# dimalit/ipt

Measured on AMD Instinct MI355X. Metric: Mpaths/sec at 1024^2, 8-bounce, sample_scenes[0]; achieved HBM GB/s, higher is better.
Workload: dtype f32; 1 GPU; c2: box 1024x1024, 1280 spp, depth_max 8, n_rays 16; width=1024, height=1024, spp=1280, depth_max=8, n_rays=16, tile_rows=0, calls=queued (ipt_render_device_async), one wait, parallelism=tiles1, per_rank=the whole frame's tiles dealt round-robin; 256 x N passes per step (weak)

## Files before the change

### ipt_amd/csrc/ipt_kernels.hip

```cpp
#include <hip/hip_runtime.h>

#include <algorithm>
#include <array>
#include <cmath>
#include <cstdio>
#include <cstdlib>
#include <cstring>
#include <strings.h>
#include <mutex>
#include <string>
#include <thread>
#include <type_traits>
#include <vector>

#include "../../include/ipt_capi.h"
#include "ipt_bvh.h"
#include "ipt_internal.h"
#include "ipt_path.h"
#include "ipt_knobs.h"
#include "ipt_diag.h"

using namespace ipt;

namespace {
// ... 52 lines not shown
    const int* __restrict__ grid_idx;
    const BvhNode* __restrict__ bvh_nodes;
    const BvhSphere* __restrict__ bvh_prims;
    int n_nodes;
    const BvhNode* __restrict__ light_nodes;
    int n_light_nodes;
    int lnodes_lds;
    const int* __restrict__ lgrid;
    const float4* __restrict__ lax;
    int lg_nu, lg_nv;
    float lg_u0, lg_v0, lg_icw, lg_ich;
    float lg_e;
    unsigned long long pk_u0, pk_u1, sa_u;
    int sa_on;
    float sa_pz, sa_nz;
    float sa_cl;
    float lg_pn, lg_nn;
    int cdf_bsearch;
    int cdf_p2;
    float cdf_p2s, cdf_end;
    int cdf_p2e;
    uint32_t cdf_end_t;
    int lpf_calc, lc_shift;
    float lc_x0, lc_y0, lc_dx, lc_dy, lc_ax, lc_ay;
    int ltr_calc, lg_ident;
    float lc_ix, lc_iy, lc_area, lc_spow;
    const int* __restrict__ cdf_lo;
    double inv_per_pass, inv_w;
    uint32_t per_pass32;
    int box_inrange;
    const float* __restrict__ cos_a;
    const float2* __restrict__ cos_b;
    const float2* __restrict__ frame_sc;
    const uint4* __restrict__ rg;
    int count;
};

__host__ __device__ inline uint32_t udiv_exact(uint32_t n, uint32_t d, double inv_d) {
    uint32_t q = (uint32_t)((double)n * inv_d);
    if (n - q * d >= d) ++q;
    return q;
}
__device__ __forceinline__ bool longer_sq(float x, float y) {
    const bool far_gt = x > y * 1.000001907f && y >= 1e-30f;
    const bool le = x <= y;
    const bool tie = !far_gt && !le;
    bool r = far_gt;
    if (__builtin_expect(__any(tie), 0))
        if (tie) r = sqrt_(x) > sqrt_(y);
    return r;
}
__device__ __forceinline__ bool longer(vec3 a, vec3 b) { return longer_sq(dot(a, a), dot(b, b)); }

__device__ __forceinline__ void vgpr_hold(float& f) { asm volatile("" : "+v"(f)); }
__device__ __forceinline__ void vgpr_hold(vec3& v) { vgpr_hold(v.x); vgpr_hold(v.y); vgpr_hold(v.z); }
__device__ __forceinline__ void vgpr_hold(int& i) { asm volatile("" : "+v"(i)); }

constexpr uint32_t kFrameTabLo = 0x3b800000u;
constexpr uint32_t kFrameTabSpan = 0x04000000u;
constexpr size_t kFrameTabEntries = 2 * ((size_t)kFrameTabSpan + 1);
__device__ __forceinline__ void frame_sc_lookup(const float2* __restrict__ tab, vec3 to, float& s, float& c) {
    const uint32_t u = f2u(to.z), m = u & 0x7fffffffu;
    const bool in = m - kFrameTabLo <= kFrameTabSpan;
    if (in) {
        const float2 e = tab[((m - kFrameTabLo) << 1) | (u >> 31)];
        s = e.x;
        c = e.y;
    }
    if (__builtin_expect(__any(!in), 0))
        if (!in) frame_angle_sc(to, &s, &c);
}

__device__ __forceinline__ bool owned_row(const KParams& kp, int yi) {
    if (kp.n_shards <= 1 || kp.tile_rows <= 0) return true;
    return ((yi / kp.tile_rows) % kp.n_shards) == kp.shard_id;
}

struct Win8 {
    uint32_t a0, a1, a2, a3, b0, b1, b2, b3;
};

__device__ __forceinline__ uint32_t sel4(uint32_t j, uint32_t x0, uint32_t x1, uint32_t x2, uint32_t x3) {
    const bool b0 = (j & 1u) != 0u, b1 = (j & 2u) != 0u;
    const uint32_t lo = b0 ? x1 : x0, hi = b0 ? x3 : x2;
    return b1 ? hi : lo;
}

__device__ __forceinline__ uint32_t cdf_threshold24(float c) {
    const float x = c * 16777216.0f;
    return !(x > 0.0f) ? 0u : (x >= 16777216.0f ? 16777216u : (uint32_t)__builtin_ceilf(x));
}

__device__ __forceinline__ void philox_fill(uint32_t& d0, uint32_t& d1, uint32_t& d2, uint32_t& d3,
                                            uint32_t blk, uint32_t pass, uint32_t pix, uint32_t k0,
                                            uint32_t k1) {
    u32x4 o = philox4x32_10(blk, pass, pix, 0u, k0, k1);
    d0 = o.v[0];
    d1 = o.v[1];
    d2 = o.v[2];
    d3 = o.v[3];
}

__device__ __forceinline__ float bvh_box_entry(const BvhNode& b, vec3 o, vec3 inv) {
    const float tx0 = (b.bmin[0] - o.x) * inv.x, tx1 = (b.bmax[0] - o.x) * inv.x;
    const float ty0 = (b.bmin[1] - o.y) * inv.y, ty1 = (b.bmax[1] - o.y) * inv.y;
    const float tz0 = (b.bmin[2] - o.z) * inv.z, tz1 = (b.bmax[2] - o.z) * inv.z;
// ... 856 lines not shown
    LightSet<LMODE> LS;
    LS.lds = lights_lds;
    LS.glob = kp.lights;
    LS.wl = global_lights(LMODE) ? gl_lds : weights_lds;
    LS.cl = global_lights(LMODE) ? cdf_gl : cdf_lds;
    LS.wg = kp.weights;
    LS.cg = kp.cdf;
    if (one_light(LMODE)) {
        LS.one = kp.lights[0];
        if (IPT_LIGHT_HOLD && (IPT_RES_HOLD || !resumable_geom(GEOM))) {
            vgpr_hold(LS.one.P); vgpr_hold(LS.one.x); vgpr_hold(LS.one.y);
            vgpr_hold(LS.one.n); vgpr_hold(LS.one.inv.c[0]); vgpr_hold(LS.one.inv.c[1]); vgpr_hold(LS.one.inv.c[2]);
        }
        LS.w0 = kp.weights[0];
        LS.c0 = kp.cdf[0];
        LS.c1 = kp.cdf[1];
    }

    auto ltrace = [&](const LightDev& L, vec3 o, vec3 d, vec3* hp, vec3* hn) -> bool {
        if constexpr (LMODE == kLightsOneA10) return light_trace_ax<1, 0, IPT_LIGHT_INR>(L, o, d, hp, hn);
        else if constexpr (LMODE == kLightsOneA01) return light_trace_ax<0, 1, IPT_LIGHT_INR>(L, o, d, hp, hn);
        else if constexpr (grid_lights(LMODE) && lattice_a10(LMODE)) return light_trace_ax<1, 0, IPT_LIGHT_INR>(L, o, d, hp, hn);
        else if constexpr (grid_lights(LMODE)) return light_trace_ax<0, 1, IPT_LIGHT_INR>(L, o, d, hp, hn);
        else return light_trace<LMODE == kLightsAny>(L, o, d, hp, hn);
    };
    auto lpdf = [&](const LightDev& L, vec3 o, bool h, vec3 hp, vec3 hn) -> float {
        if constexpr (LMODE == kLightsOneA10 || LMODE == kLightsOneA01) return light_pdf_ax<2, IPT_LIGHT_INR>(L, o, h, hp, hn);
        else if constexpr (grid_lights(LMODE)) return light_pdf_ax<2, IPT_LIGHT_INR>(L, o, h, hp, hn);
        else return light_pdf(L, o, h, hp, hn);
    };
    auto lsample = [&](const LightDev& L, vec3 o, float a, float b) -> vec3 {
        if constexpr (LMODE == kLightsOneA10) return light_sample_dir_ax<1, 0, IPT_LIGHT_INR>(L, o, a, b);
        else if constexpr (LMODE == kLightsOneA01) return light_sample_dir_ax<0, 1, IPT_LIGHT_INR>(L, o, a, b);
        else if constexpr (grid_lights(LMODE) && lattice_a10(LMODE)) return light_sample_dir_ax<1, 0, IPT_LIGHT_INR>(L, o, a, b);
        else if constexpr (grid_lights(LMODE)) return light_sample_dir_ax<0, 1, IPT_LIGHT_INR>(L, o, a, b);
        else return light_sample_dir<LMODE == kLightsAny>(L, o, a, b);
    };

    KParams kg = kp;
    if (IPT_RES_HOLD && resumable_geom(GEOM)) {
        for (int a = 0; a < 3; ++a) {
            vgpr_hold(kg.grid_g0[a]);
            vgpr_hold(kg.grid_h[a]);
            vgpr_hold(kg.grid_n[a]);
        }
        vgpr_hold(kg.grid_m);
        vgpr_hold(kg.bvh_tmargin);
    }
    const int lane = tid & 63;
    const uint64_t lanemask_lt = (lane == 0) ? 0ull : (~0ull >> (64 - lane));
    const int nl = one_light(LMODE) ? 1 : kp.n_lights;
    const float w_sdf = kp.weights[nl];
    const unsigned long long per_pass = (unsigned long long)kp.n_cand * (unsigned long long)kp.W;
    const bool n_pow2 = kp.n_rays > 0 && (kp.n_rays & (kp.n_rays - 1)) == 0;
    const int n_log2 = n_pow2 ? 31 - __clz(kp.n_rays) : 0;

    __builtin_amdgcn_s_waitcnt(0);

    unsigned long long pool_next = 0, pool_end = 0;

    bool active = true, has_path = false, fresh = false, need_frame = false, need_b = false;
    int pick = -1;
    float u1 = 0.0f, u2 = 0.0f, tr = 0.0f, cs_c = 0.0f, cs_s = 0.0f;
    float pfs = 0.0f, pfc = 0.0f;
    vec3 pto = v3(0, 0, 0);
    bool pfok = false;
    uint32_t unit = 0;
    uint32_t rpass = 0, rpix = 0, k = 0, blk = 0;
    Win8 w;
    vec3 tpos = v3(0, 0, 0);
    int fdepth = -1;
    uint32_t finm = 0;
    constexpr bool kRes = resumable_geom(GEOM);
    constexpr bool kResL = resumable_lights(LMODE, GEOM);
    constexpr int kFramePf = (kRes || kResL) ? 0 : IPT_FRAME_PF;
    constexpr bool kSkipAhead = IPT_SKIP_AHEAD && (one_light(LMODE) || grid_lights(LMODE)) && !kResL;
    constexpr bool kPreSkip = kSkipAhead && IPT_PRE_SKIP && kFramePf == 3;
    bool tracing = false;
    float xlmix = 0.0f;
    vec3 xro = v3(0, 0, 0), xrd = v3(0, 0, 0), xli_pos = v3(0, 0, 0);
    int xrdepth = 0, xi = 0, xbidx = -1;
    float xli_y = 0.0f;
    bool xis_iter = false, xhas_li = false;
    float xmult = 0.0f, xli_pow = 0.0f, xbest = 0.0f;
    vec3 xtm = v3(0, 0, 0);
    float tres = 0.0f;
    int ti = 0, tdepth = 0, tkind = 0;
    uint32_t c_paths = 0, c_traced = 0, c_surf = 0, c_light = 0, c_exp = 0, c_iter = 0,
             c_lsamp = 0, c_skip = 0, c_sframe = 0, c_ltr = 0, c_drift = 0, c_nodes = 0, c_tests = 0,
             c_lnode = 0, c_ltest = 0;
    IPT_DIAG_STATE

    for (;;) {
        IPT_STAMP_AT(0);
        const bool need = active && !has_path;
        const uint64_t needmask = __ballot(need);
        if (needmask) {
            const int cnt = __popcll(needmask);
            const int rank = __popcll(needmask & lanemask_lt);
            unsigned long long avail = pool_end - pool_next;
            unsigned long long my = 0;
            if ((unsigned long long)cnt > avail) {
                unsigned long long base = 0;
                if (lane == __ffsll((long long)needmask) - 1) {
                    base = atomicAdd(kp.unit_counter, (unsigned long long)kPoolChunk);
                    if (kp.drained && base + kPoolChunk >= kp.total_units)
                        __hip_atomic_store(kp.drained, kp.drain_seq, __ATOMIC_RELAXED, __HIP_MEMORY_SCOPE_SYSTEM);
                }
                base = __shfl(base, __ffsll((long long)needmask) - 1);
                if ((unsigned long long)rank < avail)
                    my = pool_next + rank;
                else
                    my = base + (rank - avail);
                pool_next = base + (cnt - avail);
                pool_end = base + kPoolChunk;
            } else {
                my = pool_next + rank;
                pool_next += cnt;
            }
            if (need) {
                if (my >= kp.total_units) {
                    active = false;
                } else {
                    unit = (uint32_t)my;
                    has_path = true;
                    fresh = true;
                }
            }
        }

        IPT_STAMP_AT(1);
        if (active) { IPT_PHASE(0); }
        auto pop_node = [&]() {
        if (active && has_path && !fresh && !((kRes || kResL) && tracing) && ti >= (kp.n_rays >> tdepth)) {
            IPT_PHASE(1);
            auto fin_v = [&](float r, int d) {
                float v = 0.0f;
                if (isfinite_(r))
                    v = n_pow2 ? r * __builtin_amdgcn_ldexpf(1.0f, -(n_log2 - d)) : r / (float)(kp.n_rays >> d);
                return v;
            };
            const uint32_t m = ~finm & ((1u << tdepth) - 1u);
            const int stop = m ? 31 - (int)__clz(m) : -1;
            auto lvl = [&](int l) { return stk + (size_t)(l < 0 ? 0 : l) * kStackFields * kBlock + tid; };
            const float* bs = lvl(stop);
            const float s0 = bs[0 * kBlock], s1 = bs[1 * kBlock], s2 = bs[2 * kBlock];
            const float s3 = bs[3 * kBlock], s4 = bs[4 * kBlock], s5 = bs[5 * kBlock];
            const float* b1 = lvl(tdepth - 1);
            const float r1 = b1[3 * kBlock], m1 = b1[4 * kBlock];
            const float* b2 = lvl(tdepth - 2);
            const float r2 = b2[3 * kBlock], m2 = b2[4 * kBlock];
            auto fin_s = [&](float r, int d) {
                const float q = n_pow2 ? r * __builtin_amdgcn_ldexpf(1.0f, -(n_log2 - d))
                                       : r / (float)(kp.n_rays >> (d < 0 ? 0 : d));
                return isfinite_(r) ? q : 0.0f;
            };
            float v = fin_s(tres, tdepth);
            const float v1 = fin_s(r1 + (m1 * 1.0f) * v, tdepth - 1);
            v = tdepth - 1 > stop ? v1 : v;
            const float v2 = fin_s(r2 + (m2 * 1.0f) * v, tdepth - 2);
            v = tdepth - 2 > stop ? v2 : v;
            for (int l = tdepth - 3; l > stop; --l) {
                const float* b = lvl(l);
                v = fin_v(b[3 * kBlock] + (b[4 * kBlock] * 1.0f) * v, l);
            }
            const bool resume = stop >= 0;
            const int meta = __float_as_int(s5);
            tpos = resume ? v3(s0, s1, s2) : tpos;
            tres = resume ? s3 + (s4 * 1.0f) * v : tres;
            const int mkind = (int)((uint32_t)meta >> kp.meta_shift);
            ti = resume ? meta & ((1 << kp.meta_shift) - 1) : ti;
            tkind = resume ? mkind : tkind;
            need_frame = resume ? mkind >= 5 && fdepth != stop : need_frame;
            tdepth = resume ? stop : tdepth;
            if (!resume) {
                kp.values[unit] = v >= 0.0f ? v : 0.0f;
                has_path = false;
            }
        }
        };
        if (kFramePf != 3) pop_node();

        IPT_STAMP_AT(2);
        auto frame_normal = [&]() -> vec3 {
            vec3 nrm;
            if (GEOM == IPT_GEOM_SPHERE_IN_BOX || tkind == 5) {
                nrm = tpos;
            } else {
                const float4 sp = kp.spheres[tkind - 6];
                nrm = tpos - v3(sp.x, sp.y, sp.z);
                if (GEOM == IPT_GEOM_SMALLPT && !((double)sp.w < 100.0)) nrm = -nrm;
            }
            return nrm;
        };
        constexpr bool kFrameInrange = GEOM == IPT_GEOM_SPHERE_IN_BOX;
        const bool fneed = need_frame && has_path && !fresh && !((kRes || kResL) && tracing);
        IPT_STAMP_AT(3);
        const bool iter_lane = active && has_path && !fresh && !((kRes || kResL) && tracing);
        if constexpr (kRes) {
            pick = -1;
            u1 = u2 = tr = cs_c = cs_s = 0.0f;
        }
        uint32_t gi_a = 0, gi_b = 0;
        bool gcos = false;
        uint32_t pre_w = 0u;
        bool pre_ok = false;
        vec3 lpP = v3(0, 0, 0);
        float lpx = 0.0f, lpy = 0.0f, lpn = 0.0f;
        int lptype = 0;
        auto gathers = [&](bool ran) {
            if constexpr (kRes || kResL) {
                if (ran && gcos) {
                    tr = kp.cos_a[gi_a];
                    float sp, cp;
                    sincosf_small_(two_pi_times_u24(gi_b), &sp, &cp);
                    cs_c = cp;
                    cs_s = sp;
                }
            } else {
                if constexpr (grid_lights(LMODE) && IPT_LPF && IPT_LIGHT_AX_REC) {
                    const int pk = (ran && pick >= 0 && pick < nl) ? pick : 0;
                    if (IPT_LPF_CALC && kp.lpf_calc) {
                        lpP = v3(kp.lc_x0 + (float)(pk & ((1 << kp.lc_shift) - 1)) * kp.lc_dx,
                                 kp.lc_y0 + (float)(pk >> kp.lc_shift) * kp.lc_dy, kp.lg_pn);
                        lpx = kp.lc_ax;
                        lpy = kp.lc_ay;
                    } else {
                        const float4 a = kLaxLds ? lax_lds[3 * pk] : kp.lax[3 * pk];
                        lpP = v3(a.x, a.y, kp.lg_pn);
                        lpx = a.z;
                        lpy = a.w;
                    }
                    lpn = kp.lg_nn;
                    lptype = 0;
                } else if constexpr (grid_lights(LMODE) && IPT_LPF) {
                    constexpr int XA = lattice_a10(LMODE) ? 1 : 0, YA = 1 - XA;
                    const LightDev& Ls = kp.lights[(ran && pick >= 0 && pick < nl) ? pick : 0];
                    lpP = Ls.P;
                    lpx = comp<XA>(Ls.x);
                    lpy = comp<YA>(Ls.y);
                    lpn = comp<2>(Ls.n);
                    lptype = Ls.type;
                }
                tr = kp.cos_a[gcos ? gi_a : 0u];
                if constexpr (IPT_COSB_TAB) {
                    const float2 cb = kp.cos_b[gcos ? gi_b : 0u];
                    cs_c = cb.x;
                    cs_s = cb.y;
                } else {
                    float sp, cp;
                    sincosf_small_(two_pi_times_u24(gi_b), &sp, &cp);
                    cs_c = cp;
                    cs_s = sp;
                }
            }
        };
        auto prologue = [&]() {
            if ((k >> 2) != blk) {
// ... 29 lines not shown
                        const int n0 = (c <= nl && !(r < f0)) ? 1 : 0;
                        const int n1 = (c + 1 <= nl && !(r < f1)) ? 1 : 0;
                        const int n2 = (c + 2 <= nl && !(r < f2)) ? 1 : 0;
                        const bool more = n2 != 0;
                        c += n0 + n1 + n2;
                        if (__builtin_expect(__any(more), 0))
                            if (more) while (c <= nl && !(r < LS.cdf(c))) ++c;
                    } else {
                        while (c <= nl && !(r < LS.cdf(c))) ++c;
                    }
                } else if ((global_lights(LMODE) || LMODE == kLightsAny) && kp.cdf_bsearch) {
                    int hi = nl + 1;
                    while (c < hi) {
                        const int mid = (c + hi) >> 1;
                        if (r < LS.cdf(mid)) hi = mid; else c = mid + 1;
                    }
                } else {
                    while (c <= nl && !(r < LS.cdf(c))) ++c;
                }
                return c;
            };
            auto pick_p2w = [&](uint32_t wd) {
                const uint32_t g = wd >> 8;
                const int ce = min((int)(g >> (24 - kp.cdf_p2e)), nl);
                if (kp.cdf_p2 == 2) {
                    return ce < nl ? ce : (g < kp.cdf_end_t ? nl : nl + 1);
                }
                const uint32_t fa = __float_as_uint(LS.cdf(max(ce - 1, 0))), fb = __float_as_uint(LS.cdf(ce));
                int c = (ce >= 1 && g < fa) ? ce - 1 : (g < fb ? ce : ce + 1);
                if (c >= nl) c = g < kp.cdf_end_t ? nl : nl + 1;
                return c;
            };
            constexpr bool kPickIntCdf = IPT_PICK_INT_CDF && IPT_CDF_POW2 && global_lights(LMODE);
            auto pick_word = [&](uint32_t wd) {
                if constexpr (kPickInt) return pick_w(wd);
                if constexpr (kPickIntCdf)
                    if (kp.cdf_p2) return pick_p2w(wd);
                return pick_of(u01(wd));
            };
            int c = (kPickInt || kPickIntCdf) ? pick_word(rw) : pick_of(r);
            uint32_t jj = j;
            if constexpr (kSkipAhead) {
                const bool back = (tpos.z - kp.sa_pz) * kp.sa_nz < 0.0f;
                if (kp.sa_on && c < nl && back && j <= 1u && ti + 1 < (kp.n_rays >> tdepth)) {
                    ++ti;
                    if (COUNT) { ++c_iter; ++c_lsamp; ++c_skip; }
                    k += 3;
                    jj = j + 3u;
                    c = pick_word(j == 0u ? w.a3 : w.b0);
                }
            }
            pick = c;
            if (c <= nl) {
                const bool hi = kSkipAhead && jj >= 4u;
                const uint32_t r1 = hi ? (kPreSkip && (jj & 1u) ? w.b2 : w.b1) : sel4(jj & 3u, w.a1, w.a2, w.a3, w.b0);
                const uint32_t r2 = hi ? (kPreSkip && (jj & 1u) ? w.b3 : w.b2) : sel4(jj & 3u, w.a2, w.a3, w.b0, w.b1);
                if constexpr (kPreSkip) {
                    pre_w = sel4(jj & 3u, w.a3, w.b0, w.b1, w.b2);
                    pre_ok = jj <= 3u && kp.sa_on;
                }
                u1 = u01(r1);
                u2 = u01(r2);
                if (c == nl) {
                    gi_a = r1 >> 8;
                    gi_b = r2 >> 8;
                    gcos = true;
                }
                k += 3;
            } else {
                k += 1;
            }
        };
        if (iter_lane) {
            IPT_PHASE(3);
            prologue();
        }
        gathers(iter_lane);
        if (fneed) {
            const vec3 nrm = frame_normal();
            IPT_PHASE(5);
            Frame f;
            if (IPT_FRAME_TAB && GEOM == IPT_GEOM_SPHERE_IN_BOX) {
                vec3 to;
                float fs = 0.0f, fc = 0.0f;
                if (kFramePf == 3) {
                    to = pto;
                    fs = pfs;
                    fc = pfc;
                    if constexpr (!IPT_FRAME_FB_PF) {
                    if (__builtin_expect(__any(!pfok), 0))
                        if (!pfok) {
                            to = kFrameInrange ? normalize_inrange_(nrm) : normalize(nrm);
                            frame_sc_lookup(kp.frame_sc, to, fs, fc);
                            keep_alive(fs);
                            keep_alive(fc);
                        }
                    }
                    pfok = false;
                } else {
                    to = kFrameInrange ? normalize_inrange_(nrm) : normalize(nrm);
                    frame_sc_lookup(kp.frame_sc, to, fs, fc);
                }
                if (kFrameInrange) {
                    bool ok;
                    f = make_frame_sc_fast(to, fs, fc, ok);
                    if (__builtin_expect(__any(!ok), 0))
                        if (!ok) f = make_frame_sc<kFrameInrange>(to, fs, fc);
                } else {
                    f = make_frame_sc<kFrameInrange>(to, fs, fc);
                }
            } else if (kFrameInrange) {
                f = make_frame<true>(normalize_inrange_(nrm));
            } else {
                const vec3 to = normalize(nrm);
                float fs, fc;
                if (IPT_FRAME_TAB && IPT_FRAME_TAB_LISTS && GEOM == IPT_GEOM_SPHERES_IN_BOX)
                    frame_sc_lookup(kp.frame_sc, to, fs, fc);
                else
                    frame_angle_sc(to, &fs, &fc);
                bool ok;
                f = make_frame_sc_fast(to, fs, fc, ok);
                if (__builtin_expect(__any(!ok), 0))
                    if (!ok) f = make_frame_sc<false>(to, fs, fc);
            }
            float* c = lfr + tid;
            c[0 * kFrameStride] = f.m0.x; c[1 * kFrameStride] = f.m0.y; c[2 * kFrameStride] = f.m0.z;
            c[3 * kFrameStride] = f.m1.x; c[4 * kFrameStride] = f.m1.y; c[5 * kFrameStride] = f.m1.z;
            c[6 * kFrameStride] = f.m2.x; c[7 * kFrameStride] = f.m2.y; c[8 * kFrameStride] = f.m2.z;
            c[9 * kFrameStride] = f.iz.x; c[10 * kFrameStride] = f.iz.y; c[11 * kFrameStride] = f.iz.z;
            need_frame = false;
            fdepth = tdepth;
        }
        if (IPT_PROF && wave == 0) { IPT_PHASE(11); }
        IPT_STAMP_AT(4);
        if (!__ballot(active)) break;
        IPT_STAMP_AT(5);
        const float* frc = lfr + (tkind < 5 ? kBlock + tkind : tid);

        bool have_ray = false, is_iter = false;
        vec3 ro, rd;
        int rdepth;
        if (active && has_path && fresh) {
            IPT_PHASE(2);
            fresh = false;
            if (IPT_RAYGEN) {
                uint4 r0 = kp.rg[2 * unit], r1 = kp.rg[2 * unit + 1];
                keep_alive(r0);
                keep_alive(r1);
                if (r0.w == 0u) {
                    has_path = false;
                } else {
                    ro = kp.cam_pos;
                    rd = v3(__uint_as_float(r0.x), __uint_as_float(r0.y), __uint_as_float(r0.z));
                    w.a2 = r1.x;
                    w.a3 = r1.y;
                    rpass = r1.z;
                    rpix = r1.w;
                    blk = 0;
                    need_b = true;
                    k = 2;
                    rdepth = 0;
                    have_ray = true;
                    if (COUNT) ++c_paths;
                }
            } else {
            const RayGen g = new_path_setup(kp, unit, sharded, kp.cand_rows);
            w.a0 = g.a0;
            w.a1 = g.a1;
            w.a2 = g.a2;
            w.a3 = g.a3;
            rpass = g.rpass;
            rpix = g.rpix;
            blk = 0;
            need_b = true;
            k = 2;
            if (COUNT && g.drift) ++c_drift;
            if (!g.valid) {
                has_path = false;
            } else {
                ro = kp.cam_pos;
                rd = g.rd;
                rdepth = 0;
                have_ray = true;
                if (COUNT) ++c_paths;
            }
            }
        }

        vec3 dir_bf = v3(0, 0, 0);
        constexpr bool kDirBf = one_light(LMODE);
        if constexpr (kDirBf) {
            Frame fm;
            fm.m0 = v3(frc[0 * kFrameStride], frc[1 * kFrameStride], frc[2 * kFrameStride]);
            fm.m1 = v3(frc[3 * kFrameStride], frc[4 * kFrameStride], frc[5 * kFrameStride]);
            fm.m2 = v3(frc[6 * kFrameStride], frc[7 * kFrameStride], frc[8 * kFrameStride]);
            const vec3 cdir = frame_apply(fm, v3(tr * cs_c, tr * cs_s, sqrt_inrange_(u1)));
            const vec3 ldir = lsample(LS.one, tpos, u1, u2);
            const vec3 zero = v3(0, 0, 0);
            dir_bf = pick < nl ? ldir : (pick == nl ? cdir : zero);
        }
        if (iter_lane) {
            vec3 dir = v3(0, 0, 0);
            if (kDirBf) {
                dir = dir_bf;
                if (COUNT && pick < nl) ++c_lsamp;
            } else if (pick < nl) {
                IPT_PHASE(7);
                if constexpr (grid_lights(LMODE) && IPT_LPF) {
                    constexpr int XA = lattice_a10(LMODE) ? 1 : 0, YA = 1 - XA;
                    dir = light_sample_dir_axf<XA, YA, IPT_LIGHT_INR>(lpP, lpx, lpy, lpn, lptype, tpos, u1, u2);
                } else
                dir = lsample(LS.light(pick), tpos, u1, u2);
                if (COUNT) ++c_lsamp;
            } else if (pick == nl) {
                Frame fm;
                fm.m0 = v3(frc[0 * kFrameStride], frc[1 * kFrameStride], frc[2 * kFrameStride]);
                fm.m1 = v3(frc[3 * kFrameStride], frc[4 * kFrameStride], frc[5 * kFrameStride]);
                fm.m2 = v3(frc[6 * kFrameStride], frc[7 * kFrameStride], frc[8 * kFrameStride]);
                dir = frame_apply(fm, v3(tr * cs_c, tr * cs_s, sqrt_inrange_(u1)));
            }
            ++ti;
            if (COUNT) ++c_iter;
            if (is_zero(dir)) {
                if (COUNT) ++c_skip;
            } else {
                ro = tpos;
                rd = dir;
                rdepth = tdepth + 1;
                have_ray = true;
                is_iter = true;
            }
        }
        IPT_STAMP_AT(8);
        auto resolve = [&](bool traced, float t, int prim, vec3 o, vec3 d, int depth, bool iter, float mult,
                           bool has_li, float li_y, float li_pow) {
            float cv = 0.0f;
            bool push = false;
            vec3 si_pos = v3(0, 0, 0);
            {
                const bool has_si = prim >= 0;
                if (COUNT && traced) {
                    ++c_traced;
                    c_surf += has_si ? 1u : 0u;
                    c_light += has_li ? 1u : 0u;
                }
                si_pos = o + d * t;
                const vec3 ea = si_pos - o;
                const float x = dot(ea, ea), y = li_y;
                const bool need = has_li && has_si;
                bool lg = x > y * 1.000001907f && y >= 1e-30f;
                const bool tie = need && (!lg && !(x <= y));
                if (__builtin_expect(__any(tie), 0))
                    if (tie) lg = sqrt_(x) > sqrt_(y);
                const bool li_wins = has_li && (!has_si || lg);
                const int nchild = kp.n_rays >> depth;
                const float zero = 0.0f;
                const float cv_exp = nchild == 0 ? zero / (float)nchild : 0.0f;
                cv = li_wins ? (isfinite_(li_pow) ? li_pow : 1.0f) : (has_si ? cv_exp : 0.0f);
                cv = traced ? cv : 0.0f;
                push = traced && !li_wins && has_si && nchild != 0;
                if (COUNT && traced && !li_wins && has_si) ++c_exp;
            }
            if (push) {
                IPT_PHASE(10);
                if (iter) {
                    finm = (finm & ~(1u << tdepth)) | ((ti >= (kp.n_rays >> tdepth) ? 1u : 0u) << tdepth);
                    float* b = stk + (size_t)tdepth * kStackFields * kBlock + tid;
                    b[0 * kBlock] = tpos.x;
                    b[1 * kBlock] = tpos.y;
                    b[2 * kBlock] = tpos.z;
                    b[3 * kBlock] = tres;
                    b[4 * kBlock] = mult;
                    b[5 * kBlock] = __uint_as_float((uint32_t)ti | ((uint32_t)tkind << kp.meta_shift));
                }
                tpos = si_pos;
                tkind = prim;
                if (prim >= 5) {
                    need_frame = true;
                    if (COUNT) ++c_sframe;
                }
                tres = 0.0f;
                ti = 0;
                tdepth = depth;
            } else if (iter) {
                tres = tres + (mult * 1.0f) * cv;
            } else {
                kp.values[unit] = cv >= 0.0f ? cv : 0.0f;
                has_path = false;
            }
        };
        if constexpr (kResL) {
            if (have_ray) {
                IPT_PHASE(8);
                if (COUNT) c_ltr += (uint32_t)nl * ((is_iter ? 1u : 0u) + ((rdepth < kp.depth_max) ? 1u : 0u));
                xro = ro;
                xrd = rd;
                xrdepth = rdepth;
                xis_iter = is_iter;
                xlmix = 0.0f;
                xhas_li = false;
                xli_pos = v3(0, 0, 0);
                xli_pow = 0.0f;
                xi = 0;
                tracing = true;
            }
            if (tracing) {
                if (kp.n_light_nodes > 0) {
                    const vec3 inv = v3(safe_rcp(xrd.x), safe_rcp(xrd.y), safe_rcp(xrd.z));
                    auto walk = [&](const BvhNode* __restrict__ lnodes) {
                    int budget = IPT_LWALK_BUDGET;
                    while (xi < kp.n_light_nodes && budget > 0) {
                        int leaf = -1;
                        while (xi < kp.n_light_nodes && budget > 0) {
                            --budget;
                            const BvhNode nd = lnodes[xi];
                            if (COUNT) ++c_lnode;
                            const bool enter = bvh_box_entry(nd, xro, inv) != inf_();
                            if (enter && nd.leaf >= 0) {
                                leaf = nd.leaf;
                                xi = nd.skip;
// ... 29 lines not shown
                        const bool h = light_trace<false>(L, xro, xrd, &hp, &hn);
                        if (COUNT) ++c_ltest;
                        if (xis_iter) xlmix += LS.weight(l) * light_pdf(L, xro, h, hp, hn);
                        if (h && (!xhas_li || longer(xli_pos - xro, hp - xro))) {
                            xhas_li = true;
                            xli_pos = hp;
                            xli_pow = L.spow;
                        }
                    }
                    xi = kp.n_light_nodes;
                }
                if (xi >= kp.n_light_nodes) {
                    tracing = false;
                    float mult = 0.0f;
                    if (xis_iter) {
                        const float* fc = lfr + (tkind < 5 ? kBlock + tkind : tid);
                        Frame fz;
                        fz.iz = v3(fc[9 * kFrameStride], fc[10 * kFrameStride], fc[11 * kFrameStride]);
                        const float sdf_val = frame_cosine_value(fz, xrd);
                        const float mix = xlmix + w_sdf * sdf_val;
                        mult = div_(sdf_val, mix);
                    }
                    int prim = -1;
                    float t = inf_();
                    if (xrdepth < kp.depth_max) {
                        IPT_PHASE(9);
                        t = trace_geometry<COUNT, GEOM>(kp, xro, xrd, &prim, c_nodes, c_tests);
                    }
                    const vec3 eb = xli_pos - xro;
                    resolve(xrdepth < kp.depth_max, t, prim, xro, xrd, xrdepth, xis_iter, mult, xhas_li, dot(eb, eb),
                            xli_pow);
                }
            }
        } else {
        if (have_ray) {
            IPT_PHASE(8);
            float lmix = 0.0f;
            bool has_li = false;
            vec3 li_pos = v3(0, 0, 0);
            float li_pow = 0.0f;
            float lg_ndir = 0.0f, lg_t = 0.0f;
            vec3 lg_q = v3(0, 0, 0);
            auto light_step_with = [&](const LightDev& L, float wl) {
                vec3 hp, hn;
                bool h;
                if constexpr (grid_lights(LMODE) && IPT_LIGHT_INR) {
                    constexpr int XA = lattice_a10(LMODE) ? 1 : 0, YA = 1 - XA;
                    h = light_trace_ax_q<XA, YA>(L, lg_ndir, lg_t, lg_q, &hp, &hn);
                } else {
                    h = ltrace(L, ro, rd, &hp, &hn);
                }
                if (COUNT) ++c_ltest;
                if (is_iter) lmix += wl * lpdf(L, ro, h, hp, hn);
                if (h && (!has_li || longer(li_pos - ro, hp - ro))) {
                    has_li = true;
                    li_pos = hp;
                    li_pow = L.spow;
                }
            };
            auto light_step = [&](int l) {
                if constexpr (grid_lights(LMODE) && IPT_LIGHT_AX_REC) {
                    constexpr int XA = lattice_a10(LMODE) ? 1 : 0, YA = 1 - XA;
                    float4 a, b, c;
                    if (IPT_LTR_CALC && kp.ltr_calc) {
                        a = make_float4(kp.lc_x0 + (float)(l & ((1 << kp.lc_shift) - 1)) * kp.lc_dx,
                                        kp.lc_y0 + (float)(l >> kp.lc_shift) * kp.lc_dy, kp.lc_ax, kp.lc_ay);
                        b = make_float4(kp.lc_ix, kp.lc_iy, kp.lc_area, kp.lc_spow);
                        c = make_float4(kLaxLds ? lax_lds[3 * l + 2].x : kp.lax[3 * l + 2].x, 0.0f, 0.0f, 0.0f);
                    } else if constexpr (kLaxLds) {
                        a = lax_lds[3 * l]; b = lax_lds[3 * l + 1]; c = lax_lds[3 * l + 2];
                    } else {
                        const float4* r = kp.lax + 3 * l;
                        a = r[0]; b = r[1]; c = r[2];
                    }
                    LightDev L;
                    L.P = v3(a.x, a.y, kp.lg_pn);
                    L.x = XA == 0 ? v3(a.z, 0.0f, 0.0f) : v3(0.0f, a.z, 0.0f);
                    L.y = YA == 0 ? v3(a.w, 0.0f, 0.0f) : v3(0.0f, a.w, 0.0f);
                    L.n = v3(0.0f, 0.0f, kp.lg_nn);
                    L.inv.c[XA] = v3(b.x, 0.0f, 0.0f);
                    L.inv.c[YA] = v3(0.0f, b.y, 0.0f);
                    L.inv.c[2] = v3(0.0f, 0.0f, 0.0f);
                    L.area = b.z;
                    L.spow = b.w;
                    L.type = 0;
                    L.pad = 0;
                    light_step_with(L, c.x);
                } else {
                    light_step_with(LS.light(l), LS.weight(l));
                }
            };
            if (COUNT) c_ltr += (uint32_t)nl * ((is_iter ? 1u : 0u) + ((rdepth < kp.depth_max) ? 1u : 0u));
            if constexpr (grid_lights(LMODE)) {
                constexpr int XA = lattice_a10(LMODE) ? 1 : 0, YA = 1 - XA;
                const float n_dir = kp.lg_nn * comp<2>(rd);
                const float num = kp.lg_nn * (kp.lg_pn - comp<2>(ro));
                const float t = IPT_LIGHT_INR ? div_inrange_(num, n_dir) : div_(num, n_dir);
                lg_ndir = n_dir;
                lg_t = t;
                lg_q = ro + rd * t;
                const float u = (comp<XA>(lg_q) - kp.lg_u0) * kp.lg_icw;
                const float v = (comp<YA>(lg_q) - kp.lg_v0) * kp.lg_ich;
                int cand[4] = {-1, -1, -1, -1};
                const float e = kp.lg_e;
                if (u > -1.0f && u < (float)kp.lg_nu + 1.0f && v > -1.0f && v < (float)kp.lg_nv + 1.0f) {
                    const int i0 = (int)floorf(u - e), i1 = (int)floorf(u + e);
// ... 103 lines not shown
            if (tracing && xi < 0) {
                tracing = false;
                if (IPT_GRID_WAVE != 2 && xbidx >= 0) xbidx = grid_item_index(kg, xbidx);
#if IPT_RAYLOG
                if (!COUNT && kp.raylog) {
                    const unsigned long long k = atomicAdd(kp.raylog_n, 1ull);
                    if (k % kp.raylog_every == 0 && k / kp.raylog_every < kp.raylog_cap) {
                        RayLogRec r;
                        r.o[0] = xo.x; r.o[1] = xo.y; r.o[2] = xo.z; r.t = xbest;
                        r.d[0] = xrd.x; r.d[1] = xrd.y; r.d[2] = xrd.z; r.hit = xbidx;
                        kp.raylog[k / kp.raylog_every] = r;
                    }
                }
#endif
                resolve(true, xbest, xbidx >= 0 ? 6 + xbidx : -2 - xbidx, xo, xrd, xis_iter ? tdepth + 1 : 0, xis_iter,
                        xmult, xhas_li, xli_y, xli_pow);
            }
        } else if (kRes && tracing) {
            IPT_PHASE(9);
            bool done;
            if (kp.n_grid > 0) {
                sphere_grid_walk<COUNT, IPT_GRID_PIPE != 0>(kg, xo, xrd, xi, xtm, xbest, xbidx, IPT_GRID_BUDGET, c_nodes,
                                                          c_tests IPT_DIAG_ARGS);
                done = xi < 0;
            } else {
                sphere_bvh_walk<COUNT>(kp, xo, xrd, xi, xbest, xbidx, IPT_WALK_BUDGET, c_nodes, c_tests);
                done = xi >= kp.n_nodes;
            }
            if (done) {
                tracing = false;
                if (IPT_GRID_PIPE && kp.n_grid > 0 && xbidx >= 0)
                    xbidx = grid_item_index(kg, xbidx);
                resolve(true, xbest, xbidx >= 0 ? 6 + xbidx : -2 - xbidx, xo, xrd, xis_iter ? tdepth + 1 : 0, xis_iter,
                        xmult, xhas_li, xli_y, xli_pow);
            }
        }
        }
        if constexpr (kPreSkip) {
            const bool back = (tpos.z - kp.sa_pz) * kp.sa_nz < 0.0f;
            const bool lpick = IPT_PICK_INT ? (unsigned long long)pre_w < kp.sa_u : u01(pre_w) < kp.sa_cl;
            const bool take = iter_lane && pre_ok && back && ti < (kp.n_rays >> tdepth) && lpick;
            ti += take ? 1 : 0;
            k += take ? 3u : 0u;
            if (COUNT) {
                c_iter += take ? 1u : 0u;
                c_lsamp += take ? 1u : 0u;
                c_skip += take ? 1u : 0u;
            }
        }
        if constexpr (kFramePf == 3) {
            pop_node();
            IPT_STAMP_AT(6);
            if constexpr (IPT_FRAME_TAB && kFrameInrange) {
                if (need_frame && active && has_path) {
                    const vec3 to = normalize_inrange_(tpos);
                    const uint32_t u = f2u(to.z), mz = u & 0x7fffffffu;
                    pfok = mz - kFrameTabLo <= kFrameTabSpan;
                    if (pfok) {
                        const float2 e = kp.frame_sc[((mz - kFrameTabLo) << 1) | (u >> 31)];
                        pfs = e.x;
                        pfc = e.y;
                        pto = to;
                    }
                    if constexpr (IPT_FRAME_FB_PF) {
                        if (__builtin_expect(__any(!pfok), 0))
                            if (!pfok) {
                                frame_angle_sc(to, &pfs, &pfc);
                                pto = to;
                            }
                    }
                }
            }
            IPT_STAMP_AT(7);
        }
    }

    IPT_DIAG_FLUSH(kp.counters, kNumCounters)
    if (COUNT) {
        atomicAdd(&kp.counters[0], (unsigned long long)c_paths);
        atomicAdd(&kp.counters[1], (unsigned long long)c_traced);
        atomicAdd(&kp.counters[2], (unsigned long long)c_surf);
        atomicAdd(&kp.counters[3], (unsigned long long)c_light);
        atomicAdd(&kp.counters[4], (unsigned long long)c_exp);
        atomicAdd(&kp.counters[5], (unsigned long long)c_iter);
        atomicAdd(&kp.counters[6], (unsigned long long)c_lsamp);
        atomicAdd(&kp.counters[7], (unsigned long long)c_skip);
        atomicAdd(&kp.counters[8], (unsigned long long)c_sframe);
        atomicAdd(&kp.counters[9], (unsigned long long)c_ltr);
        atomicAdd(&kp.counters[10], (unsigned long long)c_drift);
        atomicAdd(&kp.counters[11], (unsigned long long)c_nodes);
        atomicAdd(&kp.counters[12], (unsigned long long)c_tests);
        atomicAdd(&kp.counters[13], (unsigned long long)c_lnode);
        atomicAdd(&kp.counters[14], (unsigned long long)c_ltest);
    }
}

struct AParams {
    int W, H, spp, n_cand;
    const int* cand_of_row;
    const float* values;
    const uint8_t* codes;
    const uint8_t* flags;
    int tile_rows, n_shards, shard_id;
    float* pixels;
    uint32_t* counters;
    float* sums;
    float* pixel_max;
// ... 1827 lines not shown
```

### ipt_amd/csrc/ipt_path.h

```cpp
#pragma once

#include "ipt_math.h"

#include <vector>

namespace ipt {

constexpr int kMaxLights = 1024;

struct LightDev {
    vec3 P;
    vec3 x, y;
    vec3 n;
    mat3 inv;
    float area;
    float spow;
    int type;
    int pad;
};

struct Frame {
    vec3 m0, m1, m2;
    vec3 iz;
};
// ... 263 lines not shown
    return dir;
}

template <int I>
IPT_HD float comp(vec3 v) {
    return I == 0 ? v.x : (I == 1 ? v.y : v.z);
}
template <int XA, int YA>
IPT_HD bool light_trace_ax_q(const LightDev& L, float n_dir, float t, vec3 q, vec3* hit, vec3* nrm);
template <int XA, int YA, bool INR = false>
IPT_HD bool light_trace_ax(const LightDev& L, vec3 o, vec3 d, vec3* hit, vec3* nrm) {
    constexpr int NA = 3 - XA - YA;
    const float n_dir = comp<NA>(L.n) * comp<NA>(d);
    const float num = comp<NA>(L.n) * (comp<NA>(L.P) - comp<NA>(o));
    const float t = INR ? div_inrange_(num, n_dir) : div_(num, n_dir);
    return light_trace_ax_q<XA, YA>(L, n_dir, t, o + d * t, hit, nrm);
}
template <int XA, int YA>
IPT_HD bool light_trace_ax_q(const LightDev& L, float n_dir, float t, vec3 q, vec3* hit, vec3* nrm) {
    const vec3 rel = q - L.P;
    const float cx = comp<0>(L.inv.c[XA]) * comp<XA>(rel);
    const float cy = comp<1>(L.inv.c[YA]) * comp<YA>(rel);
    const bool in = L.type == 0 ? (cx >= 0.0f) & (cx <= 1.0f) & (cy >= 0.0f) & (cy <= 1.0f)
                                : (cx >= 0.0f) & (cy >= 0.0f) & (cx + cy <= 1.0f);
    *hit = L.P + rel;
    *nrm = L.n;
    return !(lt_1em6(fabs_(n_dir)) | (n_dir > 0.0f)) & !lt_1em6(t) & in;
}
template <int NA, bool INR = false>
IPT_HD float light_pdf_ax(const LightDev& L, vec3 o, bool has, vec3 hit, vec3 nrm) {
    if (!has) return 0.0f;
    const vec3 ho = hit - o;
    const float decay = dot(ho, ho);
    const float s = INR ? rcp_inrange_(sqrt_inrange_(decay))
                        : div_(1.0f, sqrt_(decay));
    const float cosinus = comp<NA>(nrm) * -(comp<NA>(ho) * s);
    const float p = INR ? div_inrange_(div_inrange_(decay, cosinus), L.area) : div_(div_(decay, cosinus), L.area);
    return cosinus < 0.0f ? 0.0f : p;
}
template <int XA, int YA, bool INR = false>
IPT_HD vec3 light_sample_dir_axf(vec3 P, float xa, float ya, float nn, int type, vec3 o, float u1, float u2raw) {
    constexpr int NA = 3 - XA - YA;
    const float u2 = u2raw * (type == 1 ? 1.0f - u1 : 1.0f);
    float pc[3];
    pc[XA] = xa * u1 + comp<XA>(P);
    pc[YA] = ya * u2 + comp<YA>(P);
    pc[NA] = comp<NA>(P);
    const vec3 dir = INR ? normalize_inrange_(v3(pc[0], pc[1], pc[2]) - o) : normalize(v3(pc[0], pc[1], pc[2]) - o);
    const float cosinus = nn * -comp<NA>(dir);
    if (cosinus < 1e-5f) return v3(0.0f, 0.0f, 0.0f);
    return dir;
}
template <int XA, int YA, bool INR = false>
IPT_HD vec3 light_sample_dir_ax(const LightDev& L, vec3 o, float u1, float u2raw) {
    constexpr int NA = 3 - XA - YA;
    const float u2 = u2raw * (L.type == 1 ? 1.0f - u1 : 1.0f);
    float pc[3];
    pc[XA] = comp<XA>(L.x) * u1 + comp<XA>(L.P);
    pc[YA] = comp<YA>(L.y) * u2 + comp<YA>(L.P);
    pc[NA] = comp<NA>(L.P);
    const vec3 dir = INR ? normalize_inrange_(v3(pc[0], pc[1], pc[2]) - o) : normalize(v3(pc[0], pc[1], pc[2]) - o);
    const float cosinus = comp<NA>(L.n) * -comp<NA>(dir);
    if (cosinus < 1e-5f) return v3(0.0f, 0.0f, 0.0f);
    return dir;
}
inline int axis_aligned_light(const LightDev& L) {
    if (L.type != 0 && L.type != 1) return 0;
    auto z = [](float f) { return (f2u(f) & 0x7fffffffu) == 0u; };
    auto one_nz = [&](vec3 v, int a) {
        const float c[3] = {v.x, v.y, v.z};
        for (int i = 0; i < 3; ++i)
            if ((i == a) == z(c[i])) return false;
        return true;
    };
    if (z(L.P.x) || z(L.P.y) || z(L.P.z)) return 0;
    const int pairs[2][2] = {{1, 0}, {0, 1}};
    for (int k = 0; k < 2; ++k) {
        const int xa = pairs[k][0], ya = pairs[k][1], na = 3 - xa - ya;
        if (!one_nz(L.x, xa) || !one_nz(L.y, ya) || !one_nz(L.n, na)) continue;
        const float r0[3] = {L.inv.c[0].x, L.inv.c[1].x, L.inv.c[2].x};
        const float r1[3] = {L.inv.c[0].y, L.inv.c[1].y, L.inv.c[2].y};
        bool ok = true;
        for (int i = 0; i < 3; ++i) {
            if (i != xa && !z(r0[i])) ok = false;
            if (i != ya && !z(r1[i])) ok = false;
        }
        if (ok) return 1 + k;
    }
    return 0;
}

inline bool light_ranges_box(const LightDev& L, int na, const float cam[3]) {
    float lo[3], hi[3];
    const float P[3] = {L.P.x, L.P.y, L.P.z}, X[3] = {L.x.x, L.x.y, L.x.z}, Y[3] = {L.y.x, L.y.y, L.y.z};
    for (int i = 0; i < 3; ++i) {
        lo[i] = P[i] + (X[i] < 0.0f ? X[i] : 0.0f) + (Y[i] < 0.0f ? Y[i] : 0.0f);
        hi[i] = P[i] + (X[i] > 0.0f ? X[i] : 0.0f) + (Y[i] > 0.0f ? Y[i] : 0.0f);
    }
    const double m = 1e-5;
    double dmin = 1e30;
    const double walls[5][2] = {{0, 1}, {1, 1}, {2, 1}, {0, -1}, {2, -1}};
    for (const auto& w : walls) {
        const int a = (int)w[0];
        const double v = w[1];
        const double dd = (lo[a] > v) ? lo[a] - v : ((hi[a] < v) ? v - hi[a] : 0.0);
        dmin = dd < dmin ? dd : dmin;
    }
    auto box_dist = [&](const double q[3]) {
        double s2 = 0.0;
        for (int i = 0; i < 3; ++i) {
            const double dd = q[i] < lo[i] ? lo[i] - q[i] : (q[i] > hi[i] ? q[i] - hi[i] : 0.0);
            s2 += dd * dd;
        }
        return __builtin_sqrt(s2);
    };
    const double origin[3] = {0, 0, 0}, c[3] = {cam[0], cam[1], cam[2]};
// ... 192 lines not shown
```

Measured before the change: 386.7 Mpaths/s.

## Micro-optimize path stack unwind, random selection and single-light sampling

Rewrites the stack pop to use explicit LDS address-space pointers with 24-bit multiplies, and replaces the ldexp scale with direct exponent-bit arithmetic. The unwind is specialized for power-of-two and non-power-of-two ray counts, and its tail loop is left un-unrolled. Other changes: a flattened select tree for random-window picks when pre-skip is on, ro unified with tpos, the frame fallback moved ahead of the copy, and the active flag dropped from several conditions. For single axis-aligned light modes it returns an ok flag instead of a zero vector and skips the nearest-hit comparison. These changes aim to cut VALU and register cost in the inner loop, but they alter control conditions (fresh/active handling) in subtle ways that could change behaviour.

```diff
diff --git a/ipt_amd/csrc/ipt_kernels.hip b/ipt_amd/csrc/ipt_kernels.hip
--- a/ipt_amd/csrc/ipt_kernels.hip
+++ b/ipt_amd/csrc/ipt_kernels.hip
@@ -128,6 +128,7 @@
 }
 __device__ __forceinline__ bool longer(vec3 a, vec3 b) { return longer_sq(dot(a, a), dot(b, b)); }
 
+typedef __attribute__((address_space(3))) float lds_float;
 __device__ __forceinline__ void vgpr_hold(float& f) { asm volatile("" : "+v"(f)); }
 __device__ __forceinline__ void vgpr_hold(vec3& v) { vgpr_hold(v.x); vgpr_hold(v.y); vgpr_hold(v.z); }
 __device__ __forceinline__ void vgpr_hold(int& i) { asm volatile("" : "+v"(i)); }
@@ -1090,8 +1091,6 @@
     const int nl = one_light(LMODE) ? 1 : kp.n_lights;
     const float w_sdf = kp.weights[nl];
     const unsigned long long per_pass = (unsigned long long)kp.n_cand * (unsigned long long)kp.W;
-    const bool n_pow2 = kp.n_rays > 0 && (kp.n_rays & (kp.n_rays - 1)) == 0;
-    const int n_log2 = n_pow2 ? 31 - __clz(kp.n_rays) : 0;
 
     __builtin_amdgcn_s_waitcnt(0);
 
@@ -1170,48 +1169,61 @@
         IPT_STAMP_AT(1);
         if (active) { IPT_PHASE(0); }
         auto pop_node = [&]() {
-        if (active && has_path && !fresh && !((kRes || kResL) && tracing) && ti >= (kp.n_rays >> tdepth)) {
+        if (has_path && (kFramePf == 3 || !fresh) && !((kRes || kResL) && tracing) && ti >= (kp.n_rays >> tdepth)) {
             IPT_PHASE(1);
-            auto fin_v = [&](float r, int d) {
-                float v = 0.0f;
-                if (isfinite_(r))
-                    v = n_pow2 ? r * __builtin_amdgcn_ldexpf(1.0f, -(n_log2 - d)) : r / (float)(kp.n_rays >> d);
-                return v;
-            };
             const uint32_t m = ~finm & ((1u << tdepth) - 1u);
             const int stop = m ? 31 - (int)__clz(m) : -1;
-            auto lvl = [&](int l) { return stk + (size_t)(l < 0 ? 0 : l) * kStackFields * kBlock + tid; };
-            const float* bs = lvl(stop);
+            constexpr int kLevelWords = kStackFields * kBlock;
+            const lds_float* sb = (const lds_float*)(stk + tid);
+            auto lvl = [&](int l) { return sb + __umul24((uint32_t)(l < 0 ? 0 : l), (uint32_t)kLevelWords); };
+            const lds_float* bs = lvl(stop);
             const float s0 = bs[0 * kBlock], s1 = bs[1 * kBlock], s2 = bs[2 * kBlock];
             const float s3 = bs[3 * kBlock], s4 = bs[4 * kBlock], s5 = bs[5 * kBlock];
-            const float* b1 = lvl(tdepth - 1);
+            const lds_float* b1 = lvl(tdepth - 1);
             const float r1 = b1[3 * kBlock], m1 = b1[4 * kBlock];
-            const float* b2 = lvl(tdepth - 2);
+            const lds_float* b2 = lvl(tdepth - 2);
             const float r2 = b2[3 * kBlock], m2 = b2[4 * kBlock];
-            auto fin_s = [&](float r, int d) {
-                const float q = n_pow2 ? r * __builtin_amdgcn_ldexpf(1.0f, -(n_log2 - d))
-                                       : r / (float)(kp.n_rays >> (d < 0 ? 0 : d));
-                return isfinite_(r) ? q : 0.0f;
+            uint32_t nr = (uint32_t)kp.n_rays;
+            asm volatile("" : "+s"(nr));
+            const bool n_pow2 = nr != 0u && (nr & (nr - 1u)) == 0u;
+            const uint32_t p2_exp = 96u + (uint32_t)__clz((int)nr);
+            float v;
+            auto unwind = [&](auto p2) {
+                constexpr bool kP2 = decltype(p2)::value;
+                const uint32_t sc0 = (p2_exp + (uint32_t)tdepth) << 23;
+                auto fin_s = [&](float r, int d, uint32_t sc) {
+                    const float q = kP2 ? r * __uint_as_float(sc) : r / (float)(kp.n_rays >> (d < 0 ? 0 : d));
+                    return isfinite_(r) ? q : 0.0f;
+                };
+                v = fin_s(tres, tdepth, sc0);
+                const float v1 = fin_s(r1 + (m1 * 1.0f) * v, tdepth - 1, sc0 - (1u << 23));
+                v = tdepth - 1 > stop ? v1 : v;
+                const float v2 = fin_s(r2 + (m2 * 1.0f) * v, tdepth - 2, sc0 - (2u << 23));
+                v = tdepth - 2 > stop ? v2 : v;
+                uint32_t sc = sc0 - (3u << 23);
+#pragma unroll 1
+                for (int l = tdepth - 3; l > stop; --l, sc -= 1u << 23) {
+                    const lds_float* b = lvl(l);
+                    const float r = b[3 * kBlock] + (b[4 * kBlock] * 1.0f) * v;
+                    v = 0.0f;
+                    if (isfinite_(r)) v = kP2 ? r * __uint_as_float(sc) : r / (float)(kp.n_rays >> l);
+                }
             };
-            float v = fin_s(tres, tdepth);
-            const float v1 = fin_s(r1 + (m1 * 1.0f) * v, tdepth - 1);
-            v = tdepth - 1 > stop ? v1 : v;
-            const float v2 = fin_s(r2 + (m2 * 1.0f) * v, tdepth - 2);
-            v = tdepth - 2 > stop ? v2 : v;
-            for (int l = tdepth - 3; l > stop; --l) {
-                const float* b = lvl(l);
-                v = fin_v(b[3 * kBlock] + (b[4 * kBlock] * 1.0f) * v, l);
-            }
-            const bool resume = stop >= 0;
-            const int meta = __float_as_int(s5);
-            tpos = resume ? v3(s0, s1, s2) : tpos;
-            tres = resume ? s3 + (s4 * 1.0f) * v : tres;
-            const int mkind = (int)((uint32_t)meta >> kp.meta_shift);
-            ti = resume ? meta & ((1 << kp.meta_shift) - 1) : ti;
-            tkind = resume ? mkind : tkind;
-            need_frame = resume ? mkind >= 5 && fdepth != stop : need_frame;
-            tdepth = resume ? stop : tdepth;
-            if (!resume) {
+            if (n_pow2)
+                unwind(std::true_type{});
+            else
+                unwind(std::false_type{});
+            if (stop >= 0) {
+                const int meta = __float_as_int(s5);
+                tpos = v3(s0, s1, s2);
+                tres = s3 + (s4 * 1.0f) * v;
+                tkind = (int)((uint32_t)meta >> kp.meta_shift);
+                ti = (int)__builtin_amdgcn_ubfe((uint32_t)meta, 0u, (uint32_t)kp.meta_shift);
+                need_frame = tkind >= 5 && fdepth != stop;
+                tdepth = stop;
+                vgpr_hold(tpos);
+                vgpr_hold(tdepth);
+            } else {
                 kp.values[unit] = v >= 0.0f ? v : 0.0f;
                 has_path = false;
             }
@@ -1234,14 +1246,14 @@
         constexpr bool kFrameInrange = GEOM == IPT_GEOM_SPHERE_IN_BOX;
         const bool fneed = need_frame && has_path && !fresh && !((kRes || kResL) && tracing);
         IPT_STAMP_AT(3);
-        const bool iter_lane = active && has_path && !fresh && !((kRes || kResL) && tracing);
+        const bool iter_lane = has_path && !fresh && !((kRes || kResL) && tracing);
         if constexpr (kRes) {
             pick = -1;
             u1 = u2 = tr = cs_c = cs_s = 0.0f;
         }
         uint32_t gi_a = 0, gi_b = 0;
         bool gcos = false;
-        uint32_t pre_w = 0u;
+        uint32_t pre_w;
         bool pre_ok = false;
         vec3 lpP = v3(0, 0, 0);
         float lpx = 0.0f, lpy = 0.0f, lpn = 0.0f;
@@ -1377,12 +1389,23 @@
             }
             pick = c;
             if (c <= nl) {
-                const bool hi = kSkipAhead && jj >= 4u;
-                const uint32_t r1 = hi ? (kPreSkip && (jj & 1u) ? w.b2 : w.b1) : sel4(jj & 3u, w.a1, w.a2, w.a3, w.b0);
-                const uint32_t r2 = hi ? (kPreSkip && (jj & 1u) ? w.b3 : w.b2) : sel4(jj & 3u, w.a2, w.a3, w.b0, w.b1);
+                uint32_t r1, r2;
                 if constexpr (kPreSkip) {
-                    pre_w = sel4(jj & 3u, w.a3, w.b0, w.b1, w.b2);
+                    const bool odd = (jj & 1u) != 0u, h0 = jj < 2u, h2 = jj >= 4u;
+                    auto sel3 = [&](uint32_t x0, uint32_t x1, uint32_t x2) {
+                        const uint32_t t = h0 ? x0 : x1;
+                        return h2 ? x2 : t;
+                    };
+                    const uint32_t e1 = sel3(w.a1, w.a3, w.b1), e2 = sel3(w.a2, w.b0, w.b2);
+                    const uint32_t e3 = sel3(w.a3, w.b1, w.b3), e4 = h0 ? w.b0 : w.b2;
+                    r1 = odd ? e2 : e1;
+                    r2 = odd ? e3 : e2;
+                    pre_w = odd ? e4 : e3;
                     pre_ok = jj <= 3u && kp.sa_on;
+                } else {
+                    const bool hi = kSkipAhead && jj >= 4u;
+                    r1 = hi ? w.b1 : sel4(jj & 3u, w.a1, w.a2, w.a3, w.b0);
+                    r2 = hi ? w.b2 : sel4(jj & 3u, w.a2, w.a3, w.b0, w.b1);
                 }
                 u1 = u01(r1);
                 u2 = u01(r2);
@@ -1409,18 +1432,18 @@
                 vec3 to;
                 float fs = 0.0f, fc = 0.0f;
                 if (kFramePf == 3) {
+                    if constexpr (!IPT_FRAME_FB_PF) {
+                    if (__builtin_expect(__any(!pfok), 0))
+                        if (!pfok) {
+                            pto = kFrameInrange ? normalize_inrange_(nrm) : normalize(nrm);
+                            frame_sc_lookup(kp.frame_sc, pto, pfs, pfc);
+                            keep_alive(pfs);
+                            keep_alive(pfc);
+                        }
+                    }
                     to = pto;
                     fs = pfs;
                     fc = pfc;
-                    if constexpr (!IPT_FRAME_FB_PF) {
-                    if (__builtin_expect(__any(!pfok), 0))
-                        if (!pfok) {
-                            to = kFrameInrange ? normalize_inrange_(nrm) : normalize(nrm);
-                            frame_sc_lookup(kp.frame_sc, to, fs, fc);
-                            keep_alive(fs);
-                            keep_alive(fc);
-                        }
-                    }
                     pfok = false;
                 } else {
                     to = kFrameInrange ? normalize_inrange_(nrm) : normalize(nrm);
@@ -1463,11 +1486,10 @@
         const float* frc = lfr + (tkind < 5 ? kBlock + tkind : tid);
 
         bool have_ray = false, is_iter = false;
-        vec3 ro, rd;
+        vec3 rd;
         int rdepth;
-        if (active && has_path && fresh) {
+        if (has_path && fresh) {
             IPT_PHASE(2);
-            fresh = false;
             if (IPT_RAYGEN) {
                 uint4 r0 = kp.rg[2 * unit], r1 = kp.rg[2 * unit + 1];
                 keep_alive(r0);
@@ -1475,7 +1497,7 @@
                 if (r0.w == 0u) {
                     has_path = false;
                 } else {
-                    ro = kp.cam_pos;
+                    tpos = kp.cam_pos;
                     rd = v3(__uint_as_float(r0.x), __uint_as_float(r0.y), __uint_as_float(r0.z));
                     w.a2 = r1.x;
                     w.a3 = r1.y;
@@ -1503,7 +1525,7 @@
             if (!g.valid) {
                 has_path = false;
             } else {
-                ro = kp.cam_pos;
+                tpos = kp.cam_pos;
                 rd = g.rd;
                 rdepth = 0;
                 have_ray = true;
@@ -1511,6 +1533,7 @@
             }
             }
         }
+        fresh = false;
 
         vec3 dir_bf = v3(0, 0, 0);
         constexpr bool kDirBf = one_light(LMODE);
@@ -1520,9 +1543,18 @@
             fm.m1 = v3(frc[3 * kFrameStride], frc[4 * kFrameStride], frc[5 * kFrameStride]);
             fm.m2 = v3(frc[6 * kFrameStride], frc[7 * kFrameStride], frc[8 * kFrameStride]);
             const vec3 cdir = frame_apply(fm, v3(tr * cs_c, tr * cs_s, sqrt_inrange_(u1)));
-            const vec3 ldir = lsample(LS.one, tpos, u1, u2);
             const vec3 zero = v3(0, 0, 0);
-            dir_bf = pick < nl ? ldir : (pick == nl ? cdir : zero);
+            if constexpr (LMODE == kLightsOneA10 || LMODE == kLightsOneA01) {
+                bool lok;
+                const vec3 ldir = LMODE == kLightsOneA10
+                                      ? light_sample_dir_ax_ok<1, 0, IPT_LIGHT_INR>(LS.one, tpos, u1, u2, &lok)
+                                      : light_sample_dir_ax_ok<0, 1, IPT_LIGHT_INR>(LS.one, tpos, u1, u2, &lok);
+                const vec3 other = pick == nl ? cdir : zero;
+                dir_bf = pick < nl && lok ? ldir : other;
+            } else {
+                const vec3 ldir = lsample(LS.one, tpos, u1, u2);
+                dir_bf = pick < nl ? ldir : (pick == nl ? cdir : zero);
+            }
         }
         if (iter_lane) {
             vec3 dir = v3(0, 0, 0);
@@ -1549,13 +1581,13 @@
             if (is_zero(dir)) {
                 if (COUNT) ++c_skip;
             } else {
-                ro = tpos;
                 rd = dir;
                 rdepth = tdepth + 1;
                 have_ray = true;
                 is_iter = true;
             }
         }
+        const vec3 ro = tpos;
         IPT_STAMP_AT(8);
         auto resolve = [&](bool traced, float t, int prim, vec3 o, vec3 d, int depth, bool iter, float mult,
                            bool has_li, float li_y, float li_pow) {
@@ -1589,8 +1621,9 @@
             if (push) {
                 IPT_PHASE(10);
                 if (iter) {
-                    finm = (finm & ~(1u << tdepth)) | ((ti >= (kp.n_rays >> tdepth) ? 1u : 0u) << tdepth);
-                    float* b = stk + (size_t)tdepth * kStackFields * kBlock + tid;
+                    const uint32_t lbit = 1u << tdepth;
+                    finm = (finm & ~lbit) | (ti >= (kp.n_rays >> tdepth) ? lbit : 0u);
+                    lds_float* b = (lds_float*)(stk + tid) + __umul24((uint32_t)tdepth, (uint32_t)(kStackFields * kBlock));
                     b[0 * kBlock] = tpos.x;
                     b[1 * kBlock] = tpos.y;
                     b[2 * kBlock] = tpos.z;
@@ -1726,6 +1759,11 @@
                 }
                 if (COUNT) ++c_ltest;
                 if (is_iter) lmix += wl * lpdf(L, ro, h, hp, hn);
+                if constexpr (LMODE == kLightsOneA10 || LMODE == kLightsOneA01) {
+                    has_li = h;
+                    li_pos = hp;
+                    li_pow = L.spow;
+                } else
                 if (h && (!has_li || longer(li_pos - ro, hp - ro))) {
                     has_li = true;
                     li_pos = hp;
@@ -1935,7 +1973,7 @@
             pop_node();
             IPT_STAMP_AT(6);
             if constexpr (IPT_FRAME_TAB && kFrameInrange) {
-                if (need_frame && active && has_path) {
+                if (need_frame && has_path) {
                     const vec3 to = normalize_inrange_(tpos);
                     const uint32_t u = f2u(to.z), mz = u & 0x7fffffffu;
                     pfok = mz - kFrameTabLo <= kFrameTabSpan;
diff --git a/ipt_amd/csrc/ipt_path.h b/ipt_amd/csrc/ipt_path.h
--- a/ipt_amd/csrc/ipt_path.h
+++ b/ipt_amd/csrc/ipt_path.h
@@ -339,7 +339,7 @@
     return dir;
 }
 template <int XA, int YA, bool INR = false>
-IPT_HD vec3 light_sample_dir_ax(const LightDev& L, vec3 o, float u1, float u2raw) {
+IPT_HD vec3 light_sample_dir_ax_ok(const LightDev& L, vec3 o, float u1, float u2raw, bool* ok) {
     constexpr int NA = 3 - XA - YA;
     const float u2 = u2raw * (L.type == 1 ? 1.0f - u1 : 1.0f);
     float pc[3];
@@ -348,7 +348,14 @@
     pc[NA] = comp<NA>(L.P);
     const vec3 dir = INR ? normalize_inrange_(v3(pc[0], pc[1], pc[2]) - o) : normalize(v3(pc[0], pc[1], pc[2]) - o);
     const float cosinus = comp<NA>(L.n) * -comp<NA>(dir);
-    if (cosinus < 1e-5f) return v3(0.0f, 0.0f, 0.0f);
+    *ok = !(cosinus < 1e-5f);
+    return dir;
+}
+template <int XA, int YA, bool INR = false>
+IPT_HD vec3 light_sample_dir_ax(const LightDev& L, vec3 o, float u1, float u2raw) {
+    bool ok;
+    const vec3 dir = light_sample_dir_ax_ok<XA, YA, INR>(L, o, u1, u2raw, &ok);
+    if (!ok) return v3(0.0f, 0.0f, 0.0f);
     return dir;
 }
 inline int axis_aligned_light(const LightDev& L) {
```

New measurement: 415.1 Mpaths/s (median of 6 runs). +7.3%, better.
